# HuiyangYu/TGSFilter

Measured on AMD Instinct MI355X. Metric: filtered Gbases/sec (end-to-end, excl. gzip I/O), higher is better.
Workload: dtype u8

## Files before the change

### tgsfilter_amd/host/pipeline.h

```cpp
#pragma once
#include <dlfcn.h>
#include <fcntl.h>
#include <malloc.h>
#include <sys/mman.h>
#include <sys/stat.h>
#include <sys/uio.h>
#include <unistd.h>
#include <zlib.h>

#include <algorithm>
#include <atomic>
#include <chrono>
#include <cmath>
#include <condition_variable>
#include <cstdio>
#include <cstring>
#include <deque>
#include <fstream>
#include <functional>
#include <iostream>
#include <map>
#include <memory>
#include <mutex>
#include <thread>
// ... 254 lines not shown
        if (fd_ < 0) return false;
        created_ = only_new;
        path_ = path;
        struct stat st;
        bool ok = fstat(fd_, &st) == 0 && S_ISREG(st.st_mode) && fallocate(fd_, 0, 0, 4096) == 0 && ftruncate(fd_, 0) == 0;
        if (ok) {
            cap_ = (virt_bytes + 4095) & ~uint64_t(4095);
            map_ = (char*)mmap(nullptr, cap_, PROT_READ | PROT_WRITE, MAP_SHARED, fd_, 0);
            ok = map_ != MAP_FAILED;
            if (ok) madvise(map_, cap_, MADV_SEQUENTIAL);
        }
        if (!ok) { ::close(fd_); fd_ = -1; if (created_) unlink(path_.c_str()); return false; }
        live() = this;
        on_die().store([] { if (MappedSink* s = live()) s->cut_back(); });
        return true;
    }
    void cut_back() {
        if (fd_ < 0) return;
        dead_.store(true);
        const uint64_t size = size_.load();
        if (created_ && size == 0) { unlink(path_.c_str()); return; }
        if (reserved_.load() > size && ftruncate(fd_, (off_t)size) != 0) {  }
    }
    uint64_t reserved() const { return reserved_.load(); }
    uint64_t planned() const { return size_.load(); }
    uint64_t capacity() const { return cap_; }
    bool reserve_to(uint64_t end, bool must = true) {
        const uint64_t have = reserved_.load();
        if (end <= have) return true;
        if (dead_.load()) return false;
        const double t0 = now_s();
        if (fallocate(fd_, 0, (off_t)have, (off_t)(end - have)) != 0) {
            if (must) die(std::string("cannot extend the output file: ") + strerror(errno));
            return false;
        }
        t_falloc += now_s() - t0;
        reserved_.store(end);
        if (dead_.load()) { cut_back(); return false; }
        return true;
    }
    void populate(uint64_t at, uint64_t n) {
        char* p = map_ + (at & ~uint64_t(4095));
        const size_t len = (size_t)(((at + n + 4095) & ~uint64_t(4095)) - (at & ~uint64_t(4095)));
        if (madvise(p, len, 23 ) != 0)
            for (size_t o = 0; o < len; o += 4096) { volatile char* q = p + o; *q = *q; }
    }
    char* place(uint64_t n) { char* p = map_ + size_.load(); size_.fetch_add(n); return p; }
    static void release(const char* p, size_t n) {
        const uintptr_t lo = ((uintptr_t)p + 4095) & ~uintptr_t(4095), hi = ((uintptr_t)p + n) & ~uintptr_t(4095);
        if (hi > lo) madvise((void*)lo, hi - lo, MADV_DONTNEED);
    }
    void close() {
        if (fd_ < 0) return;
        if (reserved_.load() != size_.load() && ftruncate(fd_, (off_t)size_.load()) != 0) die("cannot set the size of the output file");
        ::close(fd_);
        fd_ = -1;
        if (live() == this) { live() = nullptr; on_die().store(nullptr); }
    }
    bool is_open() const { return fd_ >= 0; }
    double t_falloc = 0;
private:
    static MappedSink*& live() { static MappedSink* s = nullptr; return s; }
    int fd_ = -1;
    char* map_ = nullptr;
    std::atomic<uint64_t> size_{0}, reserved_{0};
    std::atomic<bool> dead_{false};
    uint64_t cap_ = 0;
    bool created_ = false;
    std::string path_;
};

#if defined(__x86_64__)
#include <immintrin.h>
__attribute__((target("avx2"))) inline void stream_copy_avx2(char* d, const char* s, size_t n)
{
    const size_t head = (size_t)(-(uintptr_t)d & 31u) < n ? (size_t)(-(uintptr_t)d & 31u) : n;
    memcpy(d, s, head);
    d += head; s += head; n -= head;
    size_t i = 0;
    for (; i + 128 <= n; i += 128) {
        const __m256i a = _mm256_loadu_si256((const __m256i*)(s + i)), b = _mm256_loadu_si256((const __m256i*)(s + i + 32));
        const __m256i c = _mm256_loadu_si256((const __m256i*)(s + i + 64)), e = _mm256_loadu_si256((const __m256i*)(s + i + 96));
        _mm256_stream_si256((__m256i*)(d + i), a); _mm256_stream_si256((__m256i*)(d + i + 32), b);
        _mm256_stream_si256((__m256i*)(d + i + 64), c); _mm256_stream_si256((__m256i*)(d + i + 96), e);
    }
    memcpy(d + i, s + i, n - i);
}
inline void stream_copy(char* d, const char* s, size_t n)
{
    static const bool avx2 = __builtin_cpu_supports("avx2");
    if (avx2 && n >= 4096) stream_copy_avx2(d, s, n); else memcpy(d, s, n);
}
inline void stream_fence() { _mm_sfence(); }
#else
inline void stream_copy(char* d, const char* s, size_t n) { memcpy(d, s, n); }
inline void stream_fence() {}
#endif

class Pool {
public:
    explicit Pool(int n, int cpu_stage = CPU_FILL) : stage_(cpu_stage) { for (int i = 0; i < n; i++) th_.emplace_back([this] { run(); }); }
    double busy_s() { std::lock_guard<std::mutex> l(m_); return busy_; }
    void add(std::function<void()> f) {
        { std::lock_guard<std::mutex> l(m_); q_.push_back(std::move(f)); open_++; }
        cv_.notify_one();
    }
    void drain() {
        std::unique_lock<std::mutex> l(m_);
        idle_.wait(l, [&] { return open_ == 0; });
    }
    void finish() {
        { std::lock_guard<std::mutex> l(m_); stop_ = true; }
        cv_.notify_all();
        for (std::thread& t : th_) t.join();
        th_.clear();
    }
private:
    void run() {
        CpuScope cpu(stage_);
        for (;;) {
            std::function<void()> f;
            {
                std::unique_lock<std::mutex> l(m_);
                cv_.wait(l, [&] { return stop_ || !q_.empty(); });
                if (q_.empty()) return;
                f = std::move(q_.front());
                q_.pop_front();
            }
            const double t0 = now_s();
            f();
            const double dt = now_s() - t0;
            f = nullptr;
            const double dd = now_s() - t0 - dt;
            std::lock_guard<std::mutex> l(m_);
            busy_ += dt;
            destroy_ += dd;
            if (dt > longest_) longest_ = dt;
            jobs_++;
            if (first_ == 0) first_ = t0;
            last_ = std::max(last_, t0 + dt + dd);
            if (--open_ == 0) idle_.notify_all();
        }
    }
    double busy_ = 0;
    const int stage_;
public:
    double destroy_ = 0, longest_ = 0, first_ = 0, last_ = 0;
    size_t jobs_ = 0;
private:
    size_t open_ = 0;
    std::condition_variable idle_;
    std::mutex m_;
    std::condition_variable cv_;
    std::deque<std::function<void()>> q_;
    std::vector<std::thread> th_;
    bool stop_ = false;
};

class Reserver {
public:
    Reserver(MappedSink& sink, Pool& populate, uint64_t stride) : sink_(sink), pop_(populate), stride_(stride) {}
    ~Reserver() { finish(); }
    void start(uint64_t speculative_limit) {
        goal_ = speculative_limit;
        th_ = std::thread([this] { run(); });
    }
    void want(uint64_t estimate, uint64_t need) {
        std::lock_guard<std::mutex> l(m_);
        if (need > need_) need_ = need;
        goal_ = estimate > need_ ? estimate : need_;
        cv_.notify_all();
    }
    void wait_ready(uint64_t upto) {
        std::unique_lock<std::mutex> l(m_);
        ready_cv_.wait(l, [&] { return ready_ >= upto; });
    }
    void finish() {
        { std::lock_guard<std::mutex> l(m_); stop_ = true; }
        cv_.notify_all();
        if (th_.joinable()) th_.join();
    }
    double t_populate_wait = 0;
private:
    void piece_done(size_t k) {
        std::lock_guard<std::mutex> l(m_);
        done_[k] = 1;
        while (next_ < done_.size() && done_[next_]) { ready_ = ends_[next_]; next_++; }
        ready_cv_.notify_all();
    }
    void run() {
        CpuScope cpu(CPU_FALLOCATE);
        uint64_t at = 0;
        for (;;) {
            uint64_t goal, need;
            {
                std::unique_lock<std::mutex> l(m_);
                cv_.wait(l, [&] { return stop_ || goal_ > at; });
                if (stop_ && at >= need_) return;
                if (goal_ <= at) return;
                goal = stop_ ? need_ : goal_; need = need_;
            }
            uint64_t upto = std::min<uint64_t>(goal, at + stride_);
            if (upto < sink_.reserved()) upto = sink_.reserved();
            if (!sink_.reserve_to(upto, false)) {
                if (need > at) { upto = need; sink_.reserve_to(upto); }
                else { std::lock_guard<std::mutex> l(m_); goal_ = at; continue; }
            }
            const uint64_t lo = at & ~uint64_t(4095), piece = 32u << 20;
            const double d0 = now_s();
            for (uint64_t o = lo; o < upto; o += piece) {
                const uint64_t n = std::min<uint64_t>(piece, upto - o);
                size_t k;
                { std::lock_guard<std::mutex> l(m_); k = done_.size(); done_.push_back(0); ends_.push_back(o + n); }
                pop_.add([this, o, n, k] { sink_.populate(o, n); piece_done(k); });
            }
            pop_.drain();
            t_populate_wait += now_s() - d0;
            at = upto;
        }
    }
    MappedSink& sink_;
    Pool& pop_;
    const uint64_t stride_;
    std::mutex m_;
    std::condition_variable cv_, ready_cv_;
    uint64_t goal_ = 0, need_ = 0, ready_ = 0;
    std::vector<char> done_;
    std::vector<uint64_t> ends_;
    size_t next_ = 0;
    bool stop_ = false;
    std::thread th_;
};

class MappedWriter {
public:
    MappedSink sink;
    bool is_open() const { return sink.is_open(); }
    bool open(const std::string& path, uint64_t capacity, bool only_new = false) { return sink.open(path, capacity, only_new); }
    void reserve_early(uint64_t limit) {
        early_ = std::thread([this, limit] {
            CpuScope cpu(CPU_FALLOCATE);
            while (!early_stop_.load() && sink.reserved() < limit)
                if (!sink.reserve_to(std::min<uint64_t>(limit, sink.reserved() + (256u << 20)), false)) break;
        });
    }
    void start_reserving(int populate_threads, uint64_t stride, uint64_t speculative) {
        if (early_.joinable()) { early_stop_ = true; early_.join(); }
        populate_.reset(new Pool(is_open() ? populate_threads : 0, CPU_POPULATE));
        reserver_.reset(new Reserver(sink, *populate_, stride));
        if (is_open()) reserver_->start(speculative);
    }
    void start_filling(int fill_threads, uint64_t release_piece) {
        pool_.reset(new Pool(is_open() ? fill_threads : 1));
        releaser_ = std::thread([this, release_piece] {
            CpuScope cpu(CPU_RELEASER);
            for (;;) {
                const std::pair<const char*, uint64_t> r = to_release_.get();
                if (!r.first) break;
                for (uint64_t o = 0; o < r.second; o += release_piece) MappedSink::release(r.first + o, std::min<uint64_t>(release_piece, r.second - o));
            }
        });
    }
    char* claim(uint64_t n, uint64_t estimate) {
        const uint64_t end = sink.planned() + n;
        if (end > sink.capacity()) die("output more than four times the size of the input: larger than the space mapped for it (TGSF_WRITER=writev writes such a file)");
        reserver_->want(std::min<uint64_t>(std::max<uint64_t>(estimate, end), sink.capacity()), end);
        const double d0 = now_s();
        reserver_->wait_ready(end);
        t_claim_wait += now_s() - d0;
        return sink.place(n);
    }
    void fill(std::function<void()> job) { pool_->add(std::move(job)); }
    void release(const char* p, uint64_t n) { to_release_.put({p, n}); }
    void finish() {
        reserver_->finish();
        t_planned = now_s();
        pool_->finish();
        populate_->finish();
        to_release_.put({nullptr, 0});
        releaser_.join();
        t_fill_tail = now_s() - t_planned;
        sink.close();
        t_close = now_s() - t_planned - t_fill_tail;
    }
    Pool& pool() { return *pool_; }
    double t_populate_wait() const { return reserver_->t_populate_wait; }
    double t_claim_wait = 0;
    double t_planned = 0, t_fill_tail = 0, t_close = 0;
private:
    std::atomic<bool> early_stop_{false};
    std::thread early_, releaser_;
    std::unique_ptr<Pool> populate_, pool_;
    std::unique_ptr<Reserver> reserver_;
    Channel<std::pair<const char*, uint64_t>> to_release_{1 << 16};
};

}
```

### tgsfilter_amd/host/prepass.cpp

```cpp
#include "prepass.h"
#include <chrono>
#include <cstdio>

#include <unistd.h>

#include <algorithm>
#include <cstdlib>
#include <cstring>
#include <iostream>
#include <thread>
#include <unordered_map>
#include <vector>

#include "api.h"
#include "fatal.h"

namespace host {

const char* const kAdapterLib[22] = {
    "ATCTCTCTCTTTTCCTCCTCCTCCGTTGTTGTTGTTGAGAGAGAT",
    "ATCTCTCTCAACAACAACAACGGAGGAGGAGGAAAAGAGAGAGAT",
    "AAAAAAAAAAAAAAAAAATTAACGGAGGAGGAGGA",
    "TCCTCCTCCTCCGTTAATTTTTTTTTTTTTTTTTT",
    "AATGTACTTCGTTCAGTTACGTATTGCT",
// ... 10 lines not shown
    "AGCAATACGTAACTGAACGAAGTACAGGAAAAAAAA",
    "GCAATACGTAACTGAACGAAGTACAGG",
    "CCTGTACTTCGTTCAGTTACGTATTGC",
    "ACGTAACTGAACGAAGTACAGG",
    "CCTGTACTTCGTTCAGTTACGT",
    "CTTGCGGGCGGCGGACTCTCCTCTGAAGATAGAGCGACAGGCAAG",
    "CTTGCCTGTCGCTCTATCTTCAGAGGAGAGTCCGCCGCCCGCAAG",
};

std::string rev_comp(const std::string& s)
{
    static char comp[256];
    static bool init = false;
    if (!init) {
        memset(comp, 'N', sizeof comp);
        const char* a = "AGCTagctMRWSYKmrwsyk";
        const char* b = "TCGAtcgaKYWSRMkywsrm";
        for (int i = 0; a[i]; i++) comp[(unsigned char)a[i]] = b[i];
        init = true;
    }
    std::string r;
    r.reserve(s.size());
    for (size_t i = s.size(); i-- > 0;) r += comp[(unsigned char)s[i]];
    return r;
}

static int check_base_content(const std::vector<std::string>& ends, int check_len, int seq_num, float end_bias)
{
    static const struct Col { uint8_t of[256]; Col() { memset(of, 4, sizeof of); of['A'] = of['a'] = 0; of['T'] = of['t'] = 1; of['G'] = of['g'] = 2; of['C'] = of['c'] = 3; } } col;
    std::vector<int> cnt5((size_t)check_len * 5, 0);
    for (const std::string& s : ends) {
        const size_t n = std::min(s.size(), (size_t)check_len);
        for (size_t i = 0; i < n; i++) cnt5[i * 5 + col.of[(unsigned char)s[i]]]++;
    }
    std::vector<int> cnt((size_t)check_len * 4, 0);
    for (int i = 0; i < check_len; i++) for (int j = 0; j < 4; j++) cnt[(size_t)i * 4 + j] = cnt5[(size_t)i * 5 + j];
    const int max_diff = (int)((seq_num * end_bias) / 100);
    int trim = 0;
    for (int i = 1; i < check_len - 1; i++) {
        const int ld = std::min(i, 5), rd = std::min(check_len - i - 1, 5);
        bool left = false, right = false;
        for (int j = 0; j < 4; j++) {
            for (int x = 1; x <= ld; x++)
                if (abs(cnt[(size_t)i * 4 + j] - cnt[(size_t)(i - x) * 4 + j]) > max_diff) { left = true; break; }
            for (int x = 1; x <= rd; x++)
                if (abs(cnt[(size_t)(i + x) * 4 + j] - cnt[(size_t)i * 4 + j]) > max_diff) { right = true; break; }
        }
        if (left && right) trim = i + 1;
    }
    return trim;
}

static double pp_now() { return std::chrono::duration<double>(std::chrono::steady_clock::now().time_since_epoch()).count(); }
static double g_pp_create = 0, g_pp_align = 0; static int g_pp_calls = 0;

static void adapter_search(const Options& o, const std::vector<std::string>& ends, std::string& adapter, float& depth)
{
    adapter.clear(); depth = 0.f;
    float min_sim = o.mid_sim;
    if (min_sim < 0.9) min_sim = 0.9f;
    if (ends.empty()) return;

    tgsf_params p;
    memset(&p, 0, sizeof p);
    p.struct_size = sizeof p;
    p.min_len = 100; p.max_len = 2147483647; p.min_q = 0; p.max_q = 255; p.bc_len = 0;
    p.end_len = 0; p.extra_len = 0; p.end_sim = 0.75f; p.mid_sim = 0.9f; p.filter = 1; p.qtype = 33;
    p.n_adapters = 22;
    int k[22];
    size_t max_q = 0;
    for (int a = 0; a < 22; a++) {
        p.adapters[a] = kAdapterLib[a];
        p.adapter_len[a] = (int)strlen(kAdapterLib[a]);
        k[a] = (int)((1 - min_sim) * p.adapter_len[a]) + 1;
        max_q = std::max(max_q, (size_t)p.adapter_len[a]);
    }
    p.end_match_len = 2; p.mid_match_len = (int)max_q;
    const size_t per_call = 4096;
    p.max_batch_reads = (uint32_t)(per_call * 22 / (22 * 2) + 64);
    p.max_batch_bases = 1 << 20; p.max_read_len = 1 << 16;
    tgsf_ctx* ctx = nullptr;
    const double c0 = pp_now();
    if (lib().create(&p, o.devices.empty() ? o.device : o.devices[0], &ctx) != TGSF_OK) { std::cerr << "Error: " << lib().last_error(nullptr) << std::endl; quit(255); }

    g_pp_create += pp_now() - c0;
    std::unordered_map<int, int> maps;
    std::vector<uint8_t> buf; std::vector<uint64_t> off; std::vector<uint32_t> len; std::vector<uint8_t> aid;
    std::vector<int32_t> kk, res, eds;
    for (size_t b = 0; b < ends.size(); b += per_call) {
        const size_t e = std::min(ends.size(), b + per_call);
        buf.clear(); off.clear(); len.clear(); aid.clear(); kk.clear();
        for (size_t i = b; i < e; i++) {
            const uint64_t o0 = buf.size();
            buf.insert(buf.end(), ends[i].begin(), ends[i].end());
            if (ends[i].empty()) continue;
            for (int a = 0; a < 22; a++) { off.push_back(o0); len.push_back((uint32_t)ends[i].size()); aid.push_back((uint8_t)a); kk.push_back(k[a]); }
        }
        const uint32_t n = (uint32_t)off.size();
        if (!n) continue;
        res.assign((size_t)n * 4, 0); eds.assign((size_t)n * 2, 0);
        const double a0 = pp_now();
        if (lib().align_windows(ctx, buf.data(), buf.size(), off.data(), len.data(), aid.data(), kk.data(), n, res.data(), eds.data()) != TGSF_OK) {
            std::cerr << "Error: " << lib().last_error(ctx) << std::endl; quit(255);
        }
        g_pp_align += pp_now() - a0; g_pp_calls++;
        for (uint32_t i = 0; i < n; i++)
            if (res[(size_t)i * 4 + 1] > 0)
                maps[(int)aid[i]] += res[(size_t)i * 4 + 2] - res[(size_t)i * 4 + 0];
    }
    lib().destroy(ctx);
    std::vector<std::pair<int, int>> vec(maps.begin(), maps.end());
    std::sort(vec.begin(), vec.end(), [](const std::pair<int, int>& a, const std::pair<int, int>& b) { return a.second > b.second; });
    if (vec.empty()) return;
    const int best = vec.front().first;
    const std::string cand = kAdapterLib[best];
    const float mean_dep = (float)maps[best] / (float)cand.size();
    if (mean_dep >= 2 * min_sim) { adapter = cand; depth = mean_dep; }
}

PrepassResult run_prepass(Options& o, const std::function<bool(Rec&)>& next_record)
{
    PrepassResult R;
    const double t0 = pp_now();
    int check_len = std::max(std::max(o.end_len, o.bc_len), 100);
    int min_len = std::max(o.min_len, 2 * check_len);
    const int max_seq = std::max(o.ad_num, o.bc_num);
    std::vector<std::string> ends5, ends3;
    const bool need5 = o.filter && (o.head_trim < 0 || o.adapter_file.empty());
    const bool need3 = o.filter && (o.tail_trim < 0 || o.adapter_file.empty());
    int seq_num = 0, min_qc = 255, max_qc = 0;
    {
        Rec r;
        const bool has_qual = o.in_type != 0;
        while (next_record(r)) {
            const int L = (int)r.len;
            if (L < min_len) continue;
            if (seq_num >= max_seq) break;
            seq_num++;
            if (need5) ends5.emplace_back(r.seq, (size_t)check_len);
            if (need3) ends3.emplace_back(rev_comp(std::string(r.seq + (L - check_len), (size_t)check_len)));
            if (has_qual)
                for (int i = 0; i < check_len; i++) { const char c = r.qual[i]; if (min_qc > c) min_qc = c; if (max_qc < c) max_qc = c; }
        }
    }
    const double t_read = pp_now() - t0;
    if (o.in_type == 1 || o.in_type == 2) {
        if (min_qc >= 33 && min_qc <= 78 && max_qc >= 33 && max_qc <= 127) R.qtype = 33;
        else if (min_qc >= 64 && min_qc <= 108 && max_qc >= 64 && max_qc <= 127) R.qtype = 64;
        else R.qtype = min_qc < 55 ? 33 : 64;
        std::cerr << "INFO: base quality scoring: Phred" << R.qtype << std::endl;
        const int maxq = max_qc - R.qtype;
        if (o.min_q >= 0) {
            if (o.min_q >= maxq) {
                std::cerr << "Warning: max base quality score was: " << maxq << std::endl;
                std::cerr << "INFO: Please reset -q parameter." << std::endl;
                quit(255);
            }
        } else {
            if (maxq > 10 && o.read_type == "clr") o.min_q = 10;
            else if (maxq > 20 && o.read_type == "hifi") o.min_q = 20;
            else if (maxq > 10 && o.read_type == "ont") o.min_q = 10;
            else o.min_q = 0;
        }
    }
    const double t1 = pp_now();
    double t_bc = 0;
    if (o.filter) {
        {
            std::thread t3;
            if (o.tail_trim < 0) t3 = std::thread([&] { R.trim3p = check_base_content(ends3, check_len, seq_num, o.end_bias); });
            if (o.head_trim < 0) R.trim5p = check_base_content(ends5, check_len, seq_num, o.end_bias);
            if (t3.joinable()) t3.join();
        }
        if (o.head_trim < 0 && o.tail_trim < 0 && R.trim5p > o.bc_len) R.trim5p = o.bc_len;
        t_bc = pp_now() - t1;
        if (o.adapter_file.empty()) {
            adapter_search(o, ends5, R.adapter5p, R.depth5p);
            adapter_search(o, ends3, R.adapter3p, R.depth3p);
        }
    }
    if (getenv("TGSF_TIMING"))
        fprintf(stderr, "PREPASS: %d reads looked at in %.3f s | base content %.3f | adapter search %.3f (contexts %.3f, %d alignment calls %.3f)\n",
                seq_num, t_read, t_bc, pp_now() - t1 - t_bc, g_pp_create, g_pp_calls, g_pp_align);
    return R;
}

}
```

### tgsfilter_amd/host/prepass.h

```cpp
#pragma once
#include <functional>
#include <string>
#include <vector>

#include "fastx.h"
#include "options.h"

namespace host {

extern const char* const kAdapterLib[22];

std::string rev_comp(const std::string& s);

struct PrepassResult {
    int qtype = 0;
    int trim5p = 0, trim3p = 0;
    std::string adapter5p, adapter3p;
    float depth5p = 0.f, depth3p = 0.f;
};

PrepassResult run_prepass(Options& o, const std::function<bool(Rec&)>& next_record);

}
```

### tgsfilter_amd/host/run.h

```cpp
#pragma once
#include <memory>

#include "api.h"
#include "pipeline.h"
#include "prepass.h"
#include "report.h"
#include "shard.h"

namespace host {

int cpu_budget();
[[noreturn]] void leave(int code);
bool detached();

struct Run {
    explicit Run(Options& opts) : o(opts) {}

    int set_up_ranks();
    int check_file_types();
    void open_input();
    void open_output_early();
    void prepass();
    void make_contexts();
    void filter_pass();
    void downsample();
    void sum_tallies();
    void report();
    void timing_lines();

    Options& o;
    RankLink link;
    bool shard_may_use_rccl = false;
    bool sharded = false;
    bool timing = false;
    double t_epoch0 = 0, t_start = 0;
    double t_prepass = 0, t_pipe = 0, t_parse = 0, t_gpu = 0, t_write = 0, t_widle = 0, t_first = 0;

    std::string html;
    bool fasta_in = false;
    InputBytes in;
    bool streaming = false;
    size_t chunk_bytes = 64u << 20;
    int scan_threads = 1;
    size_t text_off = 0, text_size = 0;
    const char* text = nullptr;
    std::unique_ptr<RecordIndex> records_p;
    std::unique_ptr<ChunkReader> open_stream();

    std::string out_path;
    bool plain_file_out() const;
    MappedWriter mapped;
    Output out;
    bool fastq_out = false, run_filter_pass = true;

    PrepassResult pp;
    std::vector<std::string> adapters;

    uint64_t batch_text = 0;
    uint32_t batch_reads = 1u << 16;
    const Api* api = nullptr;
    double t_load = 0, t_dev = 0, t_libwait = 0;
    const RcclApi* R = nullptr;
    struct RcclUp { std::atomic<int> done{0}; int rc = TGSF_OK; std::string err; void* comm = nullptr; };
    std::shared_ptr<RcclUp> rccl_state = std::make_shared<RcclUp>();
    std::thread rccl_up;
    bool use_rccl = false;
    bool ranks_own_gpus = false;
    tgsf_params p;
    std::vector<int> ctx_dev;
    std::vector<tgsf_ctx*> ctxs;
    double t_p0 = 0;

    std::unique_ptr<Channel<std::shared_ptr<Batch>>> to_gpu, to_writer;
    std::vector<int> raw_lens, clean_lens;
    uint64_t raw_bases = 0, clean_bases = 0;
    uint64_t own_raw_bases = 0;
    std::vector<CleanRec> clean_recs;
    BatchStore store;
    std::atomic<uint64_t> stream_text{0};
    std::atomic<double> stream_share{0.0};
    std::mutex gpu_time_m;
    bool numa_bind = false;
    std::vector<int> dev_node;
    std::vector<double> dev_submit_s;
    std::vector<uint64_t> dev_bytes, dev_batches;
    int fill_threads = 1, populate_threads = 1;
    uint64_t fill_min = 1u << 20, stride_bytes = 2ull << 30;
    bool release_input = false, release_output = false;
    bool mapped_out = false;
    void reader_body();
    void feed(size_t k);
    void bind_to_node_of(size_t k);
    void writer_body();
    void fill_job(const std::shared_ptr<Batch>& b, size_t lo, size_t hi);
    void batch_done(std::shared_ptr<Batch> b);

    MappedWriter down_mapped;
    bool open_down_mapped(uint64_t capacity, uint64_t speculative);
    uint64_t down_bases = 0, down_job_recs = 0, down_job_bases = 0;
    std::vector<int> down_lens;
    std::vector<uint64_t> down_t;
    double t_dsel = 0, t_dcreate = 0, t_dqc = 0, t_dwrite = 0, t_dclose = 0, t_dsubmit = 0, t_dfirst = 0, d_kept = 0, d_span = 0;
    int n_dsubmit = 0;
    bool d_in_place = false, d_mapped = false;
    std::vector<char> select_kept();
    void second_pass(const std::vector<char>& keep);
// ... 22 lines not shown
```

### tgsfilter_amd/host/run_contexts.cpp

```cpp
#include "run.h"

namespace host {

void Run::prepass()
{
    std::unique_ptr<CpuScope> cpu_prepass(new CpuScope(CPU_PREPASS));
    if (sharded && link.rank > 0) {
    } else if (streaming) {
        std::unique_ptr<ChunkReader> cr = open_stream();
        std::shared_ptr<Chunk> ch;
        size_t at = 0;
        bool over = false;
        pp = run_prepass(o, [&](Rec& r) {
            while (!over && (!ch || at >= ch->recs.size())) {
                if (ch && !ch->message.empty()) std::cerr << ch->message << std::endl;
                if (ch && ch->last) { over = true; break; }
                ch = cr->next(o.in_file);
                at = 0;
                if (!ch) over = true;
            }
            if (over) return false;
            r = ch->recs[at++];
            return true;
        });
    } else if (sharded && link.world > 1) {
        RecordIndex whole(in.data(), in.size(), !fasta_in, std::max(scan_threads, std::min(8, cpu_budget() / 2)), 1u << 14);
        RecordIndex::Cursor cur(whole);
        pp = run_prepass(o, [&](Rec& r) { return cur.next(r); });
    } else {
        RecordIndex::Cursor cur(*records_p);
        pp = run_prepass(o, [&](Rec& r) { return cur.next(r); });
    }
    if (sharded) {
        BlobOut b;
        if (link.rank == 0) { b.pod(pp.qtype); b.pod(pp.trim5p); b.pod(pp.trim3p); b.pod(pp.depth5p); b.pod(pp.depth3p); b.pod(o.min_q); b.str(pp.adapter5p); b.str(pp.adapter3p); }
        link.bcast(b.s);
        BlobIn r(b.s);
        r.pod(pp.qtype); r.pod(pp.trim5p); r.pod(pp.trim3p); r.pod(pp.depth5p); r.pod(pp.depth3p); r.pod(o.min_q); r.str(pp.adapter5p); r.str(pp.adapter3p);
    }
    cpu_prepass.reset();
    t_prepass = now_s() - t_start;
    if (o.filter) {
        if (o.head_trim < 0) o.head_trim = pp.trim5p;
        if (o.tail_trim < 0) o.tail_trim = pp.trim3p;
        std::cerr << "INFO: trim 5' end length: " << o.head_trim << std::endl;
        std::cerr << "INFO: trim 3' end length: " << o.tail_trim << std::endl;
        std::cerr << "INFO: min output reads length: " << o.min_len << std::endl;
        if (!fasta_in) std::cerr << "INFO: min Phred average quality score: " << o.min_q << std::endl;
        auto add = [&](const std::string& a) { if (std::find(adapters.begin(), adapters.end(), a) == adapters.end()) adapters.push_back(a); };
        if (!o.adapter_file.empty()) {
            InputBytes af;
            if (af.open(o.adapter_file)) {
                const int ft = file_type(o.adapter_file);
                FastxReader rd(af.data(), af.size(), ft == 1);
                Record r;
                while (rd.next(r)) { add(std::string(r.seq)); add(rev_comp(std::string(r.seq))); }
            }
            int num = 0;
            for (const std::string& a : adapters) std::cerr << "INFO: input adapter " << ++num << " :" << a << std::endl;
        } else {
            std::string a5 = pp.adapter5p, a3 = pp.adapter3p;
            float d5 = pp.depth5p, d3 = pp.depth3p;
            if (d5 > 5 * d3) { a3.clear(); d3 = 0; } else if (d3 > 5 * d5) { a5.clear(); d5 = 0; }
            std::cerr << "INFO: 5' adapter: " << a5 << std::endl;
            std::cerr << "INFO: 3' adapter: " << a3 << std::endl;
            std::cerr << "INFO: mean depth of 5' adapter: " << d5 << std::endl;
            std::cerr << "INFO: mean depth of 3' adapter: " << d3 << std::endl;
            if (o.only_adapters) leave(0);
            if (!a5.empty()) { add(a5); add(rev_comp(a5)); }
            if (!a3.empty()) { add(a3); add(rev_comp(a3)); }
            if (a5.empty() && a3.empty()) {
                if (o.read_type == "hifi" || o.read_type == "clr") {
                    add(kAdapterLib[0]); add(kAdapterLib[1]);
                    std::cerr << "INFO: set PacBio blunt adapter to trim: " << kAdapterLib[0] << std::endl;
                } else if (o.read_type == "ont") {
                    add(kAdapterLib[8]); add(kAdapterLib[9]);
                    std::cerr << "INFO: set NanoPore rapid adapter to trim: " << kAdapterLib[8] << std::endl;
                }
            }
        }
    }
}

void Run::make_contexts()
{
    batch_text = streaming ? std::min<uint64_t>(256ull << 20, chunk_bytes)
                                    : std::min<uint64_t>(256ull << 20, std::max<uint64_t>(text_size / 8 + 4096, 1 << 16));
    if (const char* e = knob("TGSF_BATCH_BYTES")) { const long long v = atoll(e); if (v > 0) batch_text = (uint64_t)v; }
    batch_reads = 1u << 16;
    {
        uint64_t per_read = 0, cols = 0, words = 1;
// ... 95 lines not shown
```

### tgsfilter_amd/host/run_pipeline.cpp

```cpp
#include "run.h"

#include <sched.h>

namespace host {

void Run::reader_body()
{
    CpuScope cpu(CPU_BATCHER);
    if (!run_filter_pass) { for (size_t d = 0; d < ctxs.size(); d++) to_gpu->put(nullptr); return; }
    std::unique_ptr<RecordIndex::Cursor> rd;
    if (!streaming) rd.reset(new RecordIndex::Cursor(*records_p));
    std::unique_ptr<ChunkReader> cr;
    if (streaming) cr = open_stream();
    std::shared_ptr<Chunk> ch;
    size_t ch_at = 0;
    bool over = false;
    Rec r;
    auto fresh = [&] { return store.get(); };
    std::shared_ptr<Batch> b = fresh();
    const double t0 = now_s();
    double waited = 0;
    uint64_t next_id = 0;
    auto flush = [&] {
        if (b->recs.empty()) return;
// ... 103 lines not shown
        if (b->res.size() < b->recs.size()) b->res.resize(b->recs.size());
        const size_t fneed = (size_t)(b->bases / (uint64_t)std::max(p.min_len, 1)) + b->recs.size() + 16;
        if (b->frags.size() < fneed) b->frags.resize(fneed);
        const uint8_t* btext = reinterpret_cast<const uint8_t*>(b->base);
        tgsf_batch_in bi;
        memset(&bi, 0, sizeof bi);
        bi.seq = btext; bi.qual = btext;
        bi.offsets = b->off.data(); bi.qual_offsets = b->qoff.data(); bi.lengths = b->len.data();
        bi.n_reads = (uint32_t)b->recs.size(); bi.n_bytes = b->span;
        tgsf_batch_out bo{b->res.data(), b->frags.data(), (uint32_t)b->frags.size(), 0};
        if (L.submit(fctx, &bi, &bo) != TGSF_OK) die(L.last_error(fctx));
        { std::lock_guard<std::mutex> l(gpu_time_m); t_gpu += now_s() - g0; if (t_first == 0) t_first = now_s() - t_p0; }
        dev_submit_s[k] += now_s() - g0; dev_bytes[k] += b->span; dev_batches[k]++;
        b->n_frags = bo.n_frags;
        to_writer->put(std::move(b));
    }
    to_writer->put(nullptr);
}

void Run::batch_done(std::shared_ptr<Batch> b)
{
    if (b->out_bytes && release_output) mapped.release(b->dst, b->out_bytes);
    if (release_input) mapped.release(b->base, b->span);
    store.put(std::move(b));
}

void Run::filter_pass()
{
    to_gpu.reset(new Channel<std::shared_ptr<Batch>>(2 + ctxs.size()));
    to_writer.reset(new Channel<std::shared_ptr<Batch>>(256));
    if (!run_filter_pass) {
        RecordIndex::Cursor rd(*records_p);
        Rec r;
        while (rd.next(r)) {
            clean_recs.push_back({std::string_view(r.name, r.name_len), 1, r.seq, r.qual, r.len});
            clean_bases += r.len;
        }
    }

    std::thread reader([this] { reader_body(); });

    numa_bind = o.devices.size() > 1 || (link.world > 1 && ranks_own_gpus);
    if (const char* e = getenv("TGSF_NUMA")) numa_bind = atoi(e) > 0;
    dev_node.assign(ctx_dev.size(), -1);
    dev_submit_s.assign(ctx_dev.size(), 0.0);
    dev_bytes.assign(ctx_dev.size(), 0);
    dev_batches.assign(ctx_dev.size(), 0);
    std::vector<std::thread> feeders;
    for (size_t k = 0; k < ctxs.size(); k++) feeders.emplace_back([this, k] { feed(k); });

    fill_threads = std::max(1, std::min(o.n_thread, 16));
    fill_min = 1u << 20;
    if (const char* e = knob("TGSF_FILL_MIN_BYTES")) { const long long v = atoll(e); if (v > 0) fill_min = (uint64_t)v; }
    populate_threads = std::max(1, std::min(o.n_thread, 32));
    if (const char* e = knob("TGSF_POPULATE_THREADS")) { const int v = atoi(e); if (v >= 1 && v <= 64) populate_threads = v; }
    stride_bytes = streaming ? (128ull << 20) : (2ull << 30);
    if (const char* e = knob("TGSF_STRIDE_BYTES")) { const long long v = atoll(e); if (v > 0) stride_bytes = (uint64_t)v; }
    mapped.start_reserving(populate_threads, stride_bytes, (!streaming && text_size > (256u << 20)) ? (uint64_t)text_size / 4 : 0);
    {
        uint64_t early_min = 1ull << 30;
        if (const char* e = knob("TGSF_DOWN_EARLY_MIN")) early_min = strtoull(e, nullptr, 10);
        if (o.downsample && !streaming && in.mapped() && (uint64_t)text_size >= early_min) {
            uint64_t spec = (uint64_t)text_size / 4;
            if (o.genome_size > 0 && o.desired_depth > 0) spec = std::min<uint64_t>(spec, (2 * o.genome_size * (uint64_t)o.desired_depth) / (uint64_t)link.world + (uint64_t)text_size / 64);
            open_down_mapped(4 * (uint64_t)text_size + (1ull << 30), spec);
        }
    }
    const bool sync_exit = !detached();
    release_input = sync_exit && !streaming && in.mapped() && !o.downsample;
    release_output = sync_exit || streaming;
    mapped.start_filling(fill_threads, 16u << 20);
    std::thread writer([this] { writer_body(); });
    reader.join();
    for (std::thread& f : feeders) f.join();
    writer.join();
    mapped_out = mapped.is_open();
    mapped.finish();
    t_pipe = now_s() - t_p0;
}

}
```

### tgsfilter_amd/host/run_report.cpp

```cpp
#include "run.h"

#include <sys/stat.h>

namespace host {

std::vector<uint64_t> pack_rows(const std::vector<uint64_t>& v, int32_t bc2, uint32_t nb2)
{
    const size_t head = tgsf_ctr_bin_table(0, bc2, nb2);
    std::vector<uint64_t> out(v.begin(), v.begin() + (long)head);
    for (int b = 0; b < 4; b++) {
        const size_t at = tgsf_ctr_bin_table(b, bc2, nb2), n = (size_t)std::min<uint64_t>(v[TGSF_CTR_ROWS + (b >> 1)], nb2) * 5;
        out.insert(out.end(), v.begin() + (long)at, v.begin() + (long)(at + n));
    }
    return out;
}

void add_tallies(std::vector<uint64_t>& v, const std::vector<uint64_t>& part, int32_t bc2, uint32_t nb2)
{
    uint64_t rows[4];
    for (int q = 0; q < 4; q++) rows[q] = std::max(v[TGSF_CTR_ROWS + q], part[TGSF_CTR_ROWS + q]);
    const size_t head = tgsf_ctr_bin_table(0, bc2, nb2);
    for (size_t i = 0; i < head; i++) v[i] += part[i];
    for (int b = 0; b < 4; b++) {
        const size_t at = tgsf_ctr_bin_table(b, bc2, nb2), n = (size_t)std::min<uint64_t>(part[TGSF_CTR_ROWS + (b >> 1)], nb2) * 5;
// ... 203 lines not shown
            if (e.compare(0, stem.size(), stem) != 0 || e.size() == stem.size() || e.find_first_not_of("0123456789", stem.size()) != std::string::npos) continue;
            struct stat st;
            if (lstat(e.c_str(), &st) == 0 && S_ISREG(st.st_mode) && unlink(e.c_str()) == 0)
                std::cerr << "Warning: " << e << ", a part of an earlier job with more ranks, was removed." << std::endl;
        }
        for (int k = link.world; k < link.world + 1024; k++) {
            const std::string other = o.out_file + ".part" + std::to_string(k);
            struct stat st;
            if (lstat(other.c_str(), &st) != 0) { if (k >= link.world + 64) break; else continue; }
            std::cerr << "Warning: " << other << " exists and is not a part of this job (nor of an earlier one this tool listed): `cat " << o.out_file
                      << ".part*` would take it in -- the parts of this job are listed in " << list << "." << std::endl;
        }
        std::ofstream f(list, std::ios::trunc);
        f << "# tgsfilter parts, in order\n";
        for (const std::string& m : mine) f << m << "\n";
    }
    if (o.downsample && reports()) {
        if (down_lens.empty()) die("no reads to downsample");
        std::sort(down_lens.begin(), down_lens.end());
        side_stats(bc, down_lens, down_bases, tables(down_t, false), clean);
        clean.tab[8] = limit_decimals(std::round(clean.mean_qual * 1000) / 1000.0, 2);
        if (!o.filter)
            std::cerr << "INFO: " << (sharded ? down_job_recs : clean_recs.size()) << " reads with a total of " << (sharded ? down_job_bases : clean_bases) << " bases were input." << std::endl;
        std::cerr << "INFO: " << down_lens.size() << " reads with a total of " << down_bases << " bases after downsampling." << std::endl;
        if (!o.out_file.empty()) {
            if (!sharded) std::cerr << "INFO: Downsampled reads were written to: " << o.out_file << "." << std::endl;
            else std::cerr << "INFO: Downsampled reads were written to: " << o.out_file << ".part0 ... " << o.out_file << ".part" << link.world - 1
                           << " (" << link.world << " parts; concatenated in this order they are the reads in input order)." << std::endl;
        }
    }
    std::string qc = fasta_in ? "0" : "1";
    qc += o.only_qc ? "0" : ((!o.filter && o.downsample) ? "1" : "2");
    if (reports()) {
        std::ofstream ofs(html);
        write_report(ofs, qc, raw, clean);
        ofs.close();
        std::cerr << "INFO: Quality control report was written to: " << html << "." << std::endl;
    }
}

void Run::timing_lines()
{
    const Api& L = *api;
    if (timing) {
        Pool& fills = mapped.pool();
        const double t_busy = fills.busy_s();
        fprintf(stderr, "POOL: %zu jobs, busy %.3f, freeing job state %.3f, longest job %.3f, first job at %.3f, last job done at %.3f (pipeline start = 0, planner done at %.3f)\n",
                fills.jobs_, t_busy, fills.destroy_, fills.longest_, fills.first_ - t_p0, fills.last_ - t_p0, mapped.t_planned - t_p0);
        fprintf(stderr, "TIMING: total %.3f s | index+prepass %.3f | waiting for the library %.3f (load %.3f + device %.3f, beside the pre-pass) | "
                        "pipeline %.3f (batching %.3f, tgsf_submit summed over %zu feeders %.3f, plan+write %.3f, planner waiting %.3f, "
                        "first batch filtered after %.3f, fill tail %.3f, closing the output %.3f; stages overlap) | stats+report %.3f | %s (fallocate %.3f, mapping the reserved pages %.3f, fill threads busy %.3f summed)\n",
                now_s() - t_start, t_prepass, t_libwait, t_load, t_dev, t_pipe, t_parse, ctxs.size(), t_gpu, t_write, t_widle, t_first,
                mapped.t_fill_tail, mapped.t_close, now_s() - t_p0 - t_pipe, mapped_out ? "output: fallocate + mapped fill" : "output: writev", mapped.sink.t_falloc, mapped.t_populate_wait(), t_busy);
        fprintf(stderr, "RESERVE: planner waited %.3f s for pages of the output file\n", mapped.t_claim_wait);
    }
    if (timing) {
        float tot[TGSF_N_STAGES] = {0};
        uint32_t nb = 0;
        for (tgsf_ctx* c : ctxs) {
            float ms[TGSF_N_STAGES]; uint32_t n1 = 0;
            if (c && L.stage_times(c, ms, &n1) == TGSF_OK) { nb += n1; for (int i = 0; i < TGSF_N_STAGES; i++) tot[i] += ms[i]; }
        }
        double sum = 0;
        for (int i = 0; i < TGSF_N_STAGES; i++) sum += tot[i];
        char piece[256];
        snprintf(piece, sizeof piece, "GPU: kernels %.3f s summed over %zu contexts and %u batches (upper bound of the busy time: contexts overlap) = %.4f of the run |", sum * 1e-3, ctxs.size(), nb,
                 sum * 1e-3 / std::max(1e-9, now_s() - t_start));
        std::string line = piece;
        for (int i = 0; i < TGSF_N_STAGES; i++) if (tot[i] > 0) { snprintf(piece, sizeof piece, " %s %.1f ms", L.stage_name(i), tot[i]); line += piece; }
        line += "\n";
        fputs(line.c_str(), stderr);
    }
    if (timing) {
        for (size_t di = 0; di < o.devices.size(); di++) {
            if (std::find(o.devices.begin(), o.devices.begin() + (long)di, o.devices[di]) != o.devices.begin() + (long)di) continue;
            double sub = 0; uint64_t by = 0, nb2 = 0; int nf2 = 0, node = -1;
            for (size_t k = 0; k < ctx_dev.size(); k++)
                if (ctx_dev[k] == o.devices[di]) { sub += dev_submit_s[k]; by += dev_bytes[k]; nb2 += dev_batches[k]; nf2++; node = std::max(node, dev_node[k]); }
            fprintf(stderr, "DEVICE %d: %llu batches, %.2f GB of text through %d feeders, tgsf_submit %.3f s summed = %.1f GB/s per feeder, %.1f GB/s for the device over the pipeline's %.3f s%s\n",
                    o.devices[di], (unsigned long long)nb2, by * 1e-9, nf2, sub, sub > 0 ? by * 1e-9 / sub : 0.0, t_pipe > 0 ? by * 1e-9 / t_pipe : 0.0, t_pipe,
                    node >= 0 ? (" (feeders bound to NUMA node " + std::to_string(node) + ")").c_str() : "");
        }
    }
    if (timing) {
        const double proc = process_cpu_s();
        double own = 0;
        std::string line;
        char piece[160];
        for (int s = 0; s < CPU_N; s++) {
            double v = (double)cpu_ns()[s].load() * 1e-9;
            if (s == CPU_MAIN) v += (double)thread_cpu_ns() * 1e-9 - (double)cpu_ns()[CPU_PREPASS].load() * 1e-9;
            own += v;
            if (v >= 0.0005) { snprintf(piece, sizeof piece, "%s %s %.3f", line.empty() ? "" : ",", cpu_stage_name(s), v); line += piece; }
        }
        snprintf(piece, sizeof piece, "CPU: %.3f s of CPU time (user + system) for %.3f Gbases = %.4f CPU-s per Gbase |", proc, (double)own_raw_bases * 1e-9,
                 own_raw_bases ? proc / ((double)own_raw_bases * 1e-9) : 0.0);
        std::string head = piece;
        snprintf(piece, sizeof piece, " | threads of the runtime and others %.3f\n", proc - own);
        fputs((head + line + piece).c_str(), stderr);
    }
    if (timing && o.downsample)
        fprintf(stderr, "DOWN: selection %.3f | QC pass over the kept reads (%s, %.2f GB of them in %.2f GB of text): context %.3f, batches + submits %.3f (its own thread; %d submits %.3f, the first %.3f) | writing them %.3f (%s) | closing the output %.3f\n",
                t_dsel, d_in_place ? "read in place" : "packed", d_kept * 1e-9, d_span * 1e-9, t_dcreate, t_dqc, n_dsubmit, t_dsubmit, t_dfirst, t_dwrite, d_mapped ? "fallocate + threads into a mapping" : "writev", t_dclose);
    if (timing) {
        struct timespec ts; clock_gettime(CLOCK_REALTIME, &ts);
        fprintf(stderr, "CLOCK: main entered at %.6f, leaving at %.6f (epoch seconds)\n", t_epoch0, (double)ts.tv_sec + ts.tv_nsec * 1e-9);
    }
// ... 4 lines not shown
```

### tgsfilter_amd/host/run_setup.cpp

```cpp
#include "run.h"

#include <sched.h>
#include <sys/stat.h>

namespace host {

int Run::set_up_ranks()
{
    if (o.ranks >= 1 && o.shard_world > 0) { std::cerr << "Error: --ranks starts the ranks itself; --shard is for a rank started by another launcher" << std::endl; return 1; }
    if (o.ranks >= 1 || o.shard_world >= 1) {
        const int world = o.ranks >= 1 ? o.ranks : o.shard_world;
        const char* why = nullptr;
        if (o.out_file.empty() && !o.only_qc && !o.only_adapters) why = "every rank writes a part file of its own: -o is needed";
        else if (file_type(o.in_file) == 2 || (o.in_file.size() > 3 && o.in_file.compare(o.in_file.size() - 3, 3, ".gz") == 0))
            why = "the ranks take byte ranges of a plain FASTQ / FASTA text";
        if (why) { std::cerr << "Error: --ranks / --shard: " << why << std::endl; return 1; }
        if (world > 1024) { std::cerr << "Error: --ranks " << world << std::endl; return 1; }
        {
            std::vector<int> dv;
            for (int r = 0; r < world && o.ranks >= 1; r++) dv.push_back(o.devices.empty() ? r : o.devices[(size_t)r % o.devices.size()]);
            std::sort(dv.begin(), dv.end());
            shard_may_use_rccl = o.ranks < 1 || std::adjacent_find(dv.begin(), dv.end()) == dv.end();
            const char* ex = getenv("TGSF_SHARD_EXCHANGE");
            if (ex && !strcmp(ex, "socket")) shard_may_use_rccl = false;
        }
        if (o.ranks >= 1) {
            fork_ranks(world, link);
            o.device = o.devices.empty() ? link.rank : o.devices[(size_t)link.rank % o.devices.size()];
        } else {
            if (o.rendezvous.empty()) { std::cerr << "Error: --shard needs --rendezvous <path>: where the ranks of the job meet (a unix socket)" << std::endl; return 1; }
            setenv("HSA_ENABLE_IPC_MODE_LEGACY", "0", 0);
            link.rendezvous(o.shard_rank, world, o.rendezvous);
        }
        o.devices.assign(1, o.device);
        o.n_thread = std::max(2, std::min(o.n_thread, std::max(o.n_thread / world, cpu_budget() / world)));
    }
    sharded = o.ranks >= 1 || o.shard_world >= 1;
    return 0;
}

int Run::check_file_types()
{
    o.in_type = file_type(o.in_file);
    const std::string prefix = file_prefix(o.in_file);
    html = prefix + ".html";
    if (!o.out_file.empty() && !o.only_qc) {
        html = file_prefix(o.out_file) + ".html";
        o.out_type = file_type(o.out_file);
        if (file_extension(o.out_file) == "gz") o.out_gz = true;
    } else {
        o.out_type = o.fasta_out ? 0 : (o.in_type == 2 ? 1 : o.in_type);
    }
// ... 3 lines not shown
        else std::cerr << "Error: Please check your output file name: " << o.out_file << std::endl;
        return 1;
    }
    if (o.in_type == 0 && o.out_type == 1) { std::cerr << "Error: Fasta format input file can't output fastq format file" << std::endl; return 1; }
    fasta_in = o.in_type == 0;
    return 0;
}

std::unique_ptr<ChunkReader> Run::open_stream()
{
    std::string err;
    std::unique_ptr<TextSource> src = open_text(in.data(), in.size(), o.in_type == 2, err);
    if (!src) { std::cerr << "Error: " << err << " (" << o.in_file << ")" << std::endl; fflush(nullptr); _exit(255); }
    return std::unique_ptr<ChunkReader>(new ChunkReader(std::move(src), !fasta_in, chunk_bytes, 20));
}

void Run::open_input()
{
    if (o.devices.empty()) o.devices.push_back(o.device);
    lib_start(o.devices);
    if (sharded && shard_may_use_rccl) rccl_start();

    const bool coded = o.in_type == 2 || (o.in_file.size() > 3 && o.in_file.compare(o.in_file.size() - 3, 3, ".gz") == 0);
    uint64_t stream_min = 256ull << 20;
    if (const char* e = knob("TGSF_STREAM_MIN_BYTES")) stream_min = strtoull(e, nullptr, 10);
    if (coded && !o.downsample) {
        if (!in.open_raw(o.in_file)) leave(1);
        streaming = in.size() >= stream_min;
    }
    if (!streaming && !in.open(o.in_file, o.in_type == 2)) leave(1);
    chunk_bytes = [] { const char* e = knob("TGSF_CHUNK_BYTES"); return e ? (size_t)strtoull(e, nullptr, 10) : (size_t)(64u << 20); }();
    const int budget = std::max(1, cpu_budget() / link.world);
    scan_threads = std::max(1, std::min({o.n_thread, 32, std::max(2, budget / 2)}));
    text_off = 0; text_size = in.size();
    if (sharded) {
        if (streaming || (in.size() > 0 && !in.mapped())) die("--ranks / --shard: the input is not a plain text file");
        const size_t lo = find_record_start(in.data(), in.size(), (size_t)((unsigned __int128)in.size() * (unsigned)link.rank / (unsigned)link.world), !fasta_in);
        const size_t hi = link.rank + 1 == link.world ? in.size()
                        : find_record_start(in.data(), in.size(), (size_t)((unsigned __int128)in.size() * (unsigned)(link.rank + 1) / (unsigned)link.world), !fasta_in);
        text_off = lo; text_size = hi > lo ? hi - lo : 0;
    }
    text = in.data() + text_off;
    if (!streaming) records_p.reset(new RecordIndex(text, text_size, !fasta_in, scan_threads));
}

void Run::open_output_early()
{
    out_path = sharded && !o.out_file.empty() ? o.out_file + ".part" + std::to_string(link.rank) : o.out_file;
    {
        uint64_t early_min = 256ull << 20;
        if (const char* e = knob("TGSF_EARLY_OPEN_MIN")) early_min = strtoull(e, nullptr, 10);
        const bool may_map_early = plain_file_out() && !o.only_qc && !o.downsample && (o.filter || o.only_qc) &&
                                   !o.only_adapters && !streaming && in.mapped() && (uint64_t)text_size >= early_min;
        if (may_map_early && mapped.open(out_path, 4 * (uint64_t)text_size + (1ull << 30), true))
            mapped.reserve_early((uint64_t)text_size / 4);
    }
}

}
```

Measured before the change: 6.301.

## Size early output reservation from a sampled kept-share estimate; parallelize adapter searches

Replaces the fixed early fallocate thread with the full reserver, which starts at open time and populates pages. A sampler thread estimates the kept output share from a sample of records, and once the quality type is known the speculative reservation goal is resized to that estimate. The 5' and 3' adapter searches now run concurrently on two threads. The intent is to have more of the output file reserved and mapped before the filter starts claiming space, and to shorten the prepass. The cost is extra sampling work, and a wrong estimate can over-reserve space that is truncated at the end.

```diff
diff --git a/tgsfilter_amd/host/pipeline.h b/tgsfilter_amd/host/pipeline.h
--- a/tgsfilter_amd/host/pipeline.h
+++ b/tgsfilter_amd/host/pipeline.h
@@ -330,6 +330,7 @@
     }
     void close() {
         if (fd_ < 0) return;
+        if (reserved_.load() > size_.load()) cut_off = reserved_.load() - size_.load();
         if (reserved_.load() != size_.load() && ftruncate(fd_, (off_t)size_.load()) != 0) die("cannot set the size of the output file");
         ::close(fd_);
         fd_ = -1;
@@ -337,6 +338,7 @@
     }
     bool is_open() const { return fd_ >= 0; }
     double t_falloc = 0;
+    uint64_t cut_off = 0;
 private:
     static MappedSink*& live() { static MappedSink* s = nullptr; return s; }
     int fd_ = -1;
@@ -443,8 +445,15 @@
         goal_ = speculative_limit;
         th_ = std::thread([this] { run(); });
     }
+    void speculate(uint64_t goal) {
+        std::lock_guard<std::mutex> l(m_);
+        if (claimed_) return;
+        goal_ = goal;
+        cv_.notify_all();
+    }
     void want(uint64_t estimate, uint64_t need) {
         std::lock_guard<std::mutex> l(m_);
+        if (!claimed_) { claimed_ = true; t_claimed_ = now_s(); }
         if (need > need_) need_ = need;
         goal_ = estimate > need_ ? estimate : need_;
         cv_.notify_all();
@@ -459,6 +468,7 @@
         if (th_.joinable()) th_.join();
     }
     double t_populate_wait = 0;
+    double t_at_goal = 0;
 private:
     void piece_done(size_t k) {
         std::lock_guard<std::mutex> l(m_);
@@ -473,7 +483,10 @@
             uint64_t goal, need;
             {
                 std::unique_lock<std::mutex> l(m_);
+                const bool spec = !claimed_;
+                const double w0 = now_s();
                 cv_.wait(l, [&] { return stop_ || goal_ > at; });
+                if (spec) t_at_goal += (claimed_ ? t_claimed_ : now_s()) - w0;
                 if (stop_ && at >= need_) return;
                 if (goal_ <= at) return;
                 goal = stop_ ? need_ : goal_; need = need_;
@@ -506,7 +519,8 @@
     std::vector<char> done_;
     std::vector<uint64_t> ends_;
     size_t next_ = 0;
-    bool stop_ = false;
+    bool stop_ = false, claimed_ = false;
+    double t_claimed_ = 0;
     std::thread th_;
 };
 
@@ -515,15 +529,8 @@
     MappedSink sink;
     bool is_open() const { return sink.is_open(); }
     bool open(const std::string& path, uint64_t capacity, bool only_new = false) { return sink.open(path, capacity, only_new); }
-    void reserve_early(uint64_t limit) {
-        early_ = std::thread([this, limit] {
-            CpuScope cpu(CPU_FALLOCATE);
-            while (!early_stop_.load() && sink.reserved() < limit)
-                if (!sink.reserve_to(std::min<uint64_t>(limit, sink.reserved() + (256u << 20)), false)) break;
-        });
-    }
     void start_reserving(int populate_threads, uint64_t stride, uint64_t speculative) {
-        if (early_.joinable()) { early_stop_ = true; early_.join(); }
+        goal_before_claim = speculative;
         populate_.reset(new Pool(is_open() ? populate_threads : 0, CPU_POPULATE));
         reserver_.reset(new Reserver(sink, *populate_, stride));
         if (is_open()) reserver_->start(speculative);
@@ -539,8 +546,11 @@
             }
         });
     }
+    bool reserving() const { return (bool)reserver_; }
+    void speculate(uint64_t goal) { goal_before_claim = goal; reserver_->speculate(goal); }
     char* claim(uint64_t n, uint64_t estimate) {
         const uint64_t end = sink.planned() + n;
+        if (!claimed_) { claimed_ = true; reserved_at_first_claim = sink.reserved(); }
         if (end > sink.capacity()) die("output more than four times the size of the input: larger than the space mapped for it (TGSF_WRITER=writev writes such a file)");
         reserver_->want(std::min<uint64_t>(std::max<uint64_t>(estimate, end), sink.capacity()), end);
         const double d0 = now_s();
@@ -563,11 +573,13 @@
     }
     Pool& pool() { return *pool_; }
     double t_populate_wait() const { return reserver_->t_populate_wait; }
+    double t_at_goal() const { return reserver_->t_at_goal; }
+    uint64_t goal_before_claim = 0, reserved_at_first_claim = 0;
     double t_claim_wait = 0;
     double t_planned = 0, t_fill_tail = 0, t_close = 0;
 private:
-    std::atomic<bool> early_stop_{false};
-    std::thread early_, releaser_;
+    bool claimed_ = false;
+    std::thread releaser_;
     std::unique_ptr<Pool> populate_, pool_;
     std::unique_ptr<Reserver> reserver_;
     Channel<std::pair<const char*, uint64_t>> to_release_{1 << 16};
diff --git a/tgsfilter_amd/host/prepass.cpp b/tgsfilter_amd/host/prepass.cpp
--- a/tgsfilter_amd/host/prepass.cpp
+++ b/tgsfilter_amd/host/prepass.cpp
@@ -86,9 +86,9 @@
 }
 
 static double pp_now() { return std::chrono::duration<double>(std::chrono::steady_clock::now().time_since_epoch()).count(); }
-static double g_pp_create = 0, g_pp_align = 0; static int g_pp_calls = 0;
-
-static void adapter_search(const Options& o, const std::vector<std::string>& ends, std::string& adapter, float& depth)
+struct SearchTimes { double create = 0, align = 0; int calls = 0; };
+
+static void adapter_search(const Options& o, const std::vector<std::string>& ends, std::string& adapter, float& depth, SearchTimes& st)
 {
     adapter.clear(); depth = 0.f;
     float min_sim = o.mid_sim;
@@ -117,7 +117,7 @@
     const double c0 = pp_now();
     if (lib().create(&p, o.devices.empty() ? o.device : o.devices[0], &ctx) != TGSF_OK) { std::cerr << "Error: " << lib().last_error(nullptr) << std::endl; quit(255); }
 
-    g_pp_create += pp_now() - c0;
+    st.create += pp_now() - c0;
     std::unordered_map<int, int> maps;
     std::vector<uint8_t> buf; std::vector<uint64_t> off; std::vector<uint32_t> len; std::vector<uint8_t> aid;
     std::vector<int32_t> kk, res, eds;
@@ -137,7 +137,7 @@
         if (lib().align_windows(ctx, buf.data(), buf.size(), off.data(), len.data(), aid.data(), kk.data(), n, res.data(), eds.data()) != TGSF_OK) {
             std::cerr << "Error: " << lib().last_error(ctx) << std::endl; quit(255);
         }
-        g_pp_align += pp_now() - a0; g_pp_calls++;
+        st.align += pp_now() - a0; st.calls++;
         for (uint32_t i = 0; i < n; i++)
             if (res[(size_t)i * 4 + 1] > 0)
                 maps[(int)aid[i]] += res[(size_t)i * 4 + 2] - res[(size_t)i * 4 + 0];
@@ -152,7 +152,7 @@
     if (mean_dep >= 2 * min_sim) { adapter = cand; depth = mean_dep; }
 }
 
-PrepassResult run_prepass(Options& o, const std::function<bool(Rec&)>& next_record)
+PrepassResult run_prepass(Options& o, const std::function<bool(Rec&)>& next_record, const std::function<void(int qtype)>& quality_known)
 {
     PrepassResult R;
     const double t0 = pp_now();
@@ -197,8 +197,10 @@
             else o.min_q = 0;
         }
     }
+    if (quality_known) quality_known(R.qtype);
     const double t1 = pp_now();
     double t_bc = 0;
+    SearchTimes s5, s3;
     if (o.filter) {
         {
             std::thread t3;
@@ -209,13 +211,15 @@
         if (o.head_trim < 0 && o.tail_trim < 0 && R.trim5p > o.bc_len) R.trim5p = o.bc_len;
         t_bc = pp_now() - t1;
         if (o.adapter_file.empty()) {
-            adapter_search(o, ends5, R.adapter5p, R.depth5p);
-            adapter_search(o, ends3, R.adapter3p, R.depth3p);
+            (void)lib();
+            std::thread t3([&] { adapter_search(o, ends3, R.adapter3p, R.depth3p, s3); });
+            adapter_search(o, ends5, R.adapter5p, R.depth5p, s5);
+            t3.join();
         }
     }
     if (getenv("TGSF_TIMING"))
-        fprintf(stderr, "PREPASS: %d reads looked at in %.3f s | base content %.3f | adapter search %.3f (contexts %.3f, %d alignment calls %.3f)\n",
-                seq_num, t_read, t_bc, pp_now() - t1 - t_bc, g_pp_create, g_pp_calls, g_pp_align);
+        fprintf(stderr, "PREPASS: %d reads looked at in %.3f s | base content %.3f | adapter search %.3f (5' and 3' side by side; summed over both: contexts %.3f, %d alignment calls %.3f)\n",
+                seq_num, t_read, t_bc, pp_now() - t1 - t_bc, s5.create + s3.create, s5.calls + s3.calls, s5.align + s3.align);
     return R;
 }
 
diff --git a/tgsfilter_amd/host/prepass.h b/tgsfilter_amd/host/prepass.h
--- a/tgsfilter_amd/host/prepass.h
+++ b/tgsfilter_amd/host/prepass.h
@@ -19,6 +19,6 @@
     float depth5p = 0.f, depth3p = 0.f;
 };
 
-PrepassResult run_prepass(Options& o, const std::function<bool(Rec&)>& next_record);
+PrepassResult run_prepass(Options& o, const std::function<bool(Rec&)>& next_record, const std::function<void(int qtype)>& quality_known = nullptr);
 
 }
diff --git a/tgsfilter_amd/host/run.h b/tgsfilter_amd/host/run.h
--- a/tgsfilter_amd/host/run.h
+++ b/tgsfilter_amd/host/run.h
@@ -52,6 +52,13 @@
     MappedWriter mapped;
     Output out;
     bool fastq_out = false, run_filter_pass = true;
+    struct KeptSample { uint32_t len; uint64_t qual_sum, in_bytes, out_bytes; };
+    std::vector<KeptSample> sample;
+    std::thread sampler;
+    void read_sample();
+    void reserve_from_sample(int qtype);
+    double kept_share = -1;
+    void set_reserve_shape();
 
     PrepassResult pp;
     std::vector<std::string> adapters;
diff --git a/tgsfilter_amd/host/run_contexts.cpp b/tgsfilter_amd/host/run_contexts.cpp
--- a/tgsfilter_amd/host/run_contexts.cpp
+++ b/tgsfilter_amd/host/run_contexts.cpp
@@ -5,6 +5,7 @@
 void Run::prepass()
 {
     std::unique_ptr<CpuScope> cpu_prepass(new CpuScope(CPU_PREPASS));
+    const std::function<void(int)> quality_known = [this](int qtype) { reserve_from_sample(qtype); };
     if (sharded && link.rank > 0) {
     } else if (streaming) {
         std::unique_ptr<ChunkReader> cr = open_stream();
@@ -22,14 +23,14 @@
             if (over) return false;
             r = ch->recs[at++];
             return true;
-        });
+        }, quality_known);
     } else if (sharded && link.world > 1) {
         RecordIndex whole(in.data(), in.size(), !fasta_in, std::max(scan_threads, std::min(8, cpu_budget() / 2)), 1u << 14);
         RecordIndex::Cursor cur(whole);
-        pp = run_prepass(o, [&](Rec& r) { return cur.next(r); });
+        pp = run_prepass(o, [&](Rec& r) { return cur.next(r); }, quality_known);
     } else {
         RecordIndex::Cursor cur(*records_p);
-        pp = run_prepass(o, [&](Rec& r) { return cur.next(r); });
+        pp = run_prepass(o, [&](Rec& r) { return cur.next(r); }, quality_known);
     }
     if (sharded) {
         BlobOut b;
@@ -37,6 +38,7 @@
         link.bcast(b.s);
         BlobIn r(b.s);
         r.pod(pp.qtype); r.pod(pp.trim5p); r.pod(pp.trim3p); r.pod(pp.depth5p); r.pod(pp.depth3p); r.pod(o.min_q); r.str(pp.adapter5p); r.str(pp.adapter3p);
+        if (link.rank > 0) reserve_from_sample(pp.qtype);
     }
     cpu_prepass.reset();
     t_prepass = now_s() - t_start;
diff --git a/tgsfilter_amd/host/run_pipeline.cpp b/tgsfilter_amd/host/run_pipeline.cpp
--- a/tgsfilter_amd/host/run_pipeline.cpp
+++ b/tgsfilter_amd/host/run_pipeline.cpp
@@ -179,11 +179,8 @@
     fill_threads = std::max(1, std::min(o.n_thread, 16));
     fill_min = 1u << 20;
     if (const char* e = knob("TGSF_FILL_MIN_BYTES")) { const long long v = atoll(e); if (v > 0) fill_min = (uint64_t)v; }
-    populate_threads = std::max(1, std::min(o.n_thread, 32));
-    if (const char* e = knob("TGSF_POPULATE_THREADS")) { const int v = atoi(e); if (v >= 1 && v <= 64) populate_threads = v; }
-    stride_bytes = streaming ? (128ull << 20) : (2ull << 30);
-    if (const char* e = knob("TGSF_STRIDE_BYTES")) { const long long v = atoll(e); if (v > 0) stride_bytes = (uint64_t)v; }
-    mapped.start_reserving(populate_threads, stride_bytes, (!streaming && text_size > (256u << 20)) ? (uint64_t)text_size / 4 : 0);
+    set_reserve_shape();
+    if (!mapped.reserving()) mapped.start_reserving(populate_threads, stride_bytes, (!streaming && text_size > (256u << 20)) ? (uint64_t)text_size / 4 : 0);
     {
         uint64_t early_min = 1ull << 30;
         if (const char* e = knob("TGSF_DOWN_EARLY_MIN")) early_min = strtoull(e, nullptr, 10);
diff --git a/tgsfilter_amd/host/run_report.cpp b/tgsfilter_amd/host/run_report.cpp
--- a/tgsfilter_amd/host/run_report.cpp
+++ b/tgsfilter_amd/host/run_report.cpp
@@ -279,7 +279,12 @@
                         "first batch filtered after %.3f, fill tail %.3f, closing the output %.3f; stages overlap) | stats+report %.3f | %s (fallocate %.3f, mapping the reserved pages %.3f, fill threads busy %.3f summed)\n",
                 now_s() - t_start, t_prepass, t_libwait, t_load, t_dev, t_pipe, t_parse, ctxs.size(), t_gpu, t_write, t_widle, t_first,
                 mapped.t_fill_tail, mapped.t_close, now_s() - t_p0 - t_pipe, mapped_out ? "output: fallocate + mapped fill" : "output: writev", mapped.sink.t_falloc, mapped.t_populate_wait(), t_busy);
-        fprintf(stderr, "RESERVE: planner waited %.3f s for pages of the output file\n", mapped.t_claim_wait);
+        char est[96] = "no estimate of the kept share";
+        if (kept_share >= 0) snprintf(est, sizeof est, "kept share %.4f estimated from %zu sampled records", kept_share, sample.size());
+        fprintf(stderr, "RESERVE: planner waited %.3f s for pages of the output file | %s, goal %llu bytes before the first batch was planned, %llu reserved by then, "
+                        "reserver at its goal for %.3f s before that | %llu bytes cut off at the end\n",
+                mapped.t_claim_wait, est, (unsigned long long)mapped.goal_before_claim, (unsigned long long)mapped.reserved_at_first_claim,
+                mapped.t_at_goal(), (unsigned long long)mapped.sink.cut_off);
     }
     if (timing) {
         float tot[TGSF_N_STAGES] = {0};
diff --git a/tgsfilter_amd/host/run_setup.cpp b/tgsfilter_amd/host/run_setup.cpp
--- a/tgsfilter_amd/host/run_setup.cpp
+++ b/tgsfilter_amd/host/run_setup.cpp
@@ -1,3 +1,4 @@
+#include "record_out.h"
 #include "run.h"
 
 #include <sched.h>
@@ -107,9 +108,80 @@
         if (const char* e = knob("TGSF_EARLY_OPEN_MIN")) early_min = strtoull(e, nullptr, 10);
         const bool may_map_early = plain_file_out() && !o.only_qc && !o.downsample && (o.filter || o.only_qc) &&
                                    !o.only_adapters && !streaming && in.mapped() && (uint64_t)text_size >= early_min;
-        if (may_map_early && mapped.open(out_path, 4 * (uint64_t)text_size + (1ull << 30), true))
-            mapped.reserve_early((uint64_t)text_size / 4);
+        if (may_map_early && mapped.open(out_path, 4 * (uint64_t)text_size + (1ull << 30), true)) {
+            set_reserve_shape();
+            mapped.start_reserving(populate_threads, stride_bytes, (uint64_t)text_size / 4);
+            const char* e = knob("TGSF_EARLY_ESTIMATE");
+            if (!(e && e[0] == '0')) sampler = std::thread([this] { read_sample(); });
+        }
     }
 }
 
+void Run::set_reserve_shape()
+{
+    populate_threads = std::max(1, std::min(o.n_thread, 32));
+    if (const char* e = knob("TGSF_POPULATE_THREADS")) { const int v = atoi(e); if (v >= 1 && v <= 64) populate_threads = v; }
+    stride_bytes = streaming ? (128ull << 20) : (2ull << 30);
+    if (const char* e = knob("TGSF_STRIDE_BYTES")) { const long long v = atoll(e); if (v > 0) stride_bytes = (uint64_t)v; }
 }
+
+static constexpr double kReserveOfEstimate = 0.9;
+static constexpr size_t kSampleRecords = 500, kSampleMinRecords = 32;
+static constexpr uint64_t kSampleQualBytes = 64ull << 20;
+
+void Run::read_sample()
+{
+    CpuScope cpu(CPU_PREPASS);
+    const size_t max_seq = (size_t)std::max(1, std::max(o.ad_num, o.bc_num));
+    const char* const text_end = text + text_size;
+    const bool fq_out = o.out_type == 1;
+    auto walk = [&](size_t m, size_t& seen) {
+        sample.clear();
+        uint64_t qual_bytes = 0;
+        Rec r, nx;
+        for (seen = 0; seen < max_seq && qual_bytes < kSampleQualBytes && records_p->get(seen, r); seen += m) {
+            KeptSample k{r.len, 0, 0, 0};
+            k.in_bytes = (uint64_t)((records_p->get(seen + 1, nx) ? nx.name - 1 : text_end) - (r.name - 1));
+            k.out_bytes = record_bytes(CleanRec{std::string_view(r.name, r.name_len), 1, r.seq, r.qual, r.len}, fq_out);
+            if (!fasta_in) {
+                const unsigned char* q = (const unsigned char*)r.qual;
+                uint64_t sum = 0;
+                for (uint32_t i = 0; i < r.len; i++) sum += q[i];
+                k.qual_sum = sum;
+                qual_bytes += r.len;
+            }
+            sample.push_back(k);
+        }
+    };
+    size_t seen = 0;
+    const size_t m0 = std::max<size_t>(1, max_seq / kSampleRecords);
+    walk(m0, seen);
+    Rec r;
+    if (m0 > 1 && sample.size() < kSampleRecords / 2 && seen < max_seq && !records_p->get(seen, r)) {
+        const size_t n = records_p->wait_complete();
+        walk(std::max<size_t>(1, std::min(n, max_seq) / kSampleRecords), seen);
+    }
+}
+
+void Run::reserve_from_sample(int qtype)
+{
+    if (!sampler.joinable()) return;
+    sampler.join();
+    if (sample.size() < kSampleMinRecords) return;
+    const double min_q = o.min_q < 0 ? 0.0 : (double)o.min_q, max_q = (double)o.max_q;
+    uint64_t in_bytes = 0, kept_bytes = 0;
+    for (const KeptSample& k : sample) {
+        in_bytes += k.in_bytes;
+        if (k.len == 0 || (int64_t)k.len < (int64_t)o.min_len || (int64_t)k.len > (int64_t)o.max_len) continue;
+        if (!fasta_in) {
+            const double mean = ((double)k.qual_sum - (double)qtype * (double)k.len) / (double)k.len;
+            if (mean < min_q || mean > max_q) continue;
+        }
+        kept_bytes += k.out_bytes;
+    }
+    if (!in_bytes) return;
+    kept_share = (double)kept_bytes / (double)in_bytes;
+    mapped.speculate((uint64_t)std::min((double)text_size, kReserveOfEstimate * kept_share * (double)text_size));
+}
+
+}
```

Measured after the change: 6.312 (median of 2 runs). About the same (+0.2%).
